# uci-cbcl/RP-Net

Hardware: AMD Instinct MI355X
Metric: support/query pairs/sec (fwd+bwd, 1-shot 256x256, T=5) (higher is better)
Workload: dtype f32

## Files before the change

### rpnet_amd/csrc/conv_wgrad_ring.hip

```cpp
#include <type_traits>

#include "common.h"
#include "lds_dma.h"
#include "split_bf16.h"

namespace rpnet {

using s16x4r = __attribute__((ext_vector_type(4))) short;
typedef __attribute__((address_space(3))) s16x4r lds_s16x4r_t;

template <int N, int I = 0, typename F>
__device__ __forceinline__ void static_for_r(F&& f) {
    if constexpr (I < N) {
        f(std::integral_constant<int, I>{});
        static_for_r<N, I + 1>(f);
    }
}

template <bool K64, int ABL = 0, int LA = 5, int NSY = 6, bool BI = false>
__global__ __launch_bounds__(256, 1) void conv_wgrad9_ring_kernel(const rpnet_conv_desc d, const unsigned short* __restrict__ dy,
                                                                   float* __restrict__ partial, const int M, const int Cin,
                                                                   const int Cout, const int tiles, const int tiles_n,
                                                                   const int ksplit, const int steps_per_split, const int lw,
                                                                   const int lh) {
    constexpr int NP = 2, BK = 32, RB = 128;
    constexpr int A_PLANE = BK * RB, A_STRIP = NP * A_PLANE;
    constexpr int NSX = 8, ZOFF = NSX * A_STRIP;
    constexpr int ZROW = 40, B_PLANE = 48 * RB, B_STAGE = NP * B_PLANE;
    constexpr int NS = NSY, BOFF = ZOFF + A_STRIP;
    static_assert(LA >= 2 && LA <= 5 && LA % NSY >= 2, "the DMAs of step st + LA must not land in a slot / stage that step st or st + 1 reads");
    __shared__ __attribute__((aligned(1024))) unsigned char smem[BOFF + NS * B_STAGE];
    RPNET_ASSERT_NO_CORESIDENCE(sizeof(smem));
    constexpr int PXS = K64 ? 64 : BK;

    const int t = threadIdx.x;
    const int lane = t & 63;
    const int wv = __builtin_amdgcn_readfirstlane(t >> 6);
    const int wm = wv >> 1, wn = wv & 1;
    int tile, z;
    const int xg = ksplit < 8 ? 8 / max(ksplit, 1) : 0;
    if ((ksplit & 7) == 0) {
        const int xcd = blockIdx.x & 7, j = blockIdx.x >> 3;
        const int jt = uni(j / tiles);
        z = jt * 8 + xcd;
        tile = j - jt * tiles;
    } else if (xg * ksplit == 8 && tiles % xg == 0) {
        const int xcd = blockIdx.x & 7, j = blockIdx.x >> 3;
        z = uni(xcd / xg);
        tile = (xcd - z * xg) * (tiles / xg) + j;
    } else {
        z = uni(blockIdx.x / tiles);
        tile = blockIdx.x - z * tiles;
    }
    const int tm = uni(tile / tiles_n), tn = tile - tm * tiles_n;
    const int cm0 = tm * 64, n0 = tn * 64;

    const int H = d.H, W = d.W;
    const unsigned short* src; int Cs, cc;
    if (cm0 < d.C0) { src = reinterpret_cast<const unsigned short*>(d.x0); Cs = d.C0; cc = cm0; }
    else { src = reinterpret_cast<const unsigned short*>(d.x1); Cs = d.C1; cc = cm0 - d.C0; }
    const size_t planex = (size_t)d.N * H * W * Cs, planey = (size_t)M * Cout;
    const int pbx = (int)(planex * 2), pby = (int)(planey * 2);

    const int total_steps = M / PXS;
    const int s_begin = z * steps_per_split;
    const int s_end = min(s_begin + steps_per_split, total_steps);
    const int lxb = lw - (K64 ? 6 : 5), xbm = (1 << lxb) - 1;
    auto q0_of = [&](const int s) {
        const int col = s >> lh, y = s & (H - 1);
        return ((((col >> lxb) << lh) + y) << lw) + (col & xbm) * PXS;
    };

    const srd_t rsx = make_srd(src, (K64 ? 1 : NP) * pbx), rsy = make_srd(dy, (K64 ? 1 : NP) * pby);
    const int x_slot1 = K64 ? BK * (Cs * 2) : pbx, y_slot1 = K64 ? BK * (Cout * 2) : pby;
    const __amdgpu_buffer_rsrc_t bix = __builtin_amdgcn_make_buffer_rsrc(const_cast<unsigned short*>(src), (short)0, (K64 ? 1 : NP) * pbx, 0x00020000);
    const __amdgpu_buffer_rsrc_t biy = __builtin_amdgcn_make_buffer_rsrc(const_cast<unsigned short*>(dy), (short)0, (K64 ? 1 : NP) * pby, 0x00020000);
    auto dma16 = [&](const bool is_x, const unsigned base, auto offc, const int voff, const int soff) {
        constexpr int OFF = decltype(offc)::value;
        if constexpr (BI) {
            auto* lp = (__attribute__((address_space(3))) void*)(smem + (base - lds_addr(smem)) + OFF);
            if (is_x) __builtin_amdgcn_raw_ptr_buffer_load_lds(bix, lp, 16, voff, soff, 0, 0);
            else __builtin_amdgcn_raw_ptr_buffer_load_lds(biy, lp, 16, voff, soff, 0, 0);
        } else if constexpr (OFF == 0) {
            lds_dma16(is_x ? rsx : rsy, base, voff, soff);
        } else {
            lds_dma16_at<OFF>(is_x ? rsx : rsy, base, voff, soff);
        }
    };
    const unsigned lds0 = lds_addr(smem);
    const unsigned ldsw = lds0 + 8 * wv * RB;
    const unsigned lds4 = lds0 + 32 * RB + (wv & 1) * B_PLANE;

    const int drow = lane >> 3;
    const int dcol = ((((lane >> 2) & 1) ^ ((lane >> 4) & 1)) << 6) | ((lane & 3) << 4);
    const int Cs2 = Cs * 2;
    const int xlane = drow * Cs2 + dcol;
    auto dma_x = [&](const int slot, const int rs) {
        if constexpr (ABL == 2 || ABL == 4) return;
        const int soff = (q0_of(rs) + 8 * wv) * Cs2 + cc * 2;
        const unsigned dst = ldsw + (slot & (NSX - 1)) * A_STRIP;
        dma16(true, dst, std::integral_constant<int, 0>{}, xlane, soff);
        dma16(true, dst, std::integral_constant<int, A_PLANE>{}, xlane, soff + x_slot1);
    };
    const int ylane = drow * (Cout * 2) + dcol, ylane_m1 = ylane - Cout * 2;
    auto dma_y = [&](auto stagec, const int st) {
        constexpr int stage = decltype(stagec)::value;
        constexpr int DST = BOFF + stage * B_STAGE;
        if constexpr (ABL == 2 || ABL == 4) return;
        const int rowb = q0_of(st) - 1 + 8 * wv;
        const bool neg = rowb < 0;
        const int soff = (neg ? 0 : rowb) * (Cout * 2) + n0 * 2;
        int voff = neg ? ylane_m1 : ylane;
        voff = rowb + drow < M ? voff : (int)0x80000000;
        const int soff1 = K64 ? (rowb + BK) * (Cout * 2) + n0 * 2 : soff + y_slot1;
        const int voff1 = K64 ? (rowb + BK + drow < M ? ylane : (int)0x80000000) : voff;
        dma16(false, ldsw, std::integral_constant<int, DST>{}, voff, soff);
        dma16(false, ldsw, std::integral_constant<int, DST + B_PLANE>{}, voff1, soff1);
    };
    auto dma_y5 = [&](auto stagec, const int st) {
        constexpr int stage = decltype(stagec)::value;
        constexpr int DST = BOFF + stage * B_STAGE;
        if constexpr (ABL == 2 || ABL == 4) return;
        const int rowb = q0_of(st) + 31 + (K64 ? wv * BK : 0);
        const int soff = rowb * (Cout * 2) + n0 * 2 + (K64 ? 0 : wv * y_slot1);
        const int voff = rowb + drow < M ? ylane : (int)0x80000000;
        dma16(false, lds4, std::integral_constant<int, DST>{}, voff, soff);
    };
    const int xlast = total_steps - 1;
    auto stc = [&](const int st) { return st < s_end ? st : s_end - 1; };
    auto xsc = [&](const int r) { return r < xlast ? r : xlast; };
    auto wait_all_but_one_step = [&]() {
        if constexpr (ABL == 2 || ABL == 4 || ABL >= 5) return;
        asm volatile("s_waitcnt vmcnt(%0)" ::"n"((LA - 2) * 4) : "memory");
    };

    {
        const u32x4 zero = {0u, 0u, 0u, 0u};
        *reinterpret_cast<u32x4*>(smem + ZOFF + t * 16) = zero;
        *reinterpret_cast<u32x4*>(smem + ZOFF + 4096 + t * 16) = zero;
        if (t < NS * NP * 8) {
            const int pl = t >> 3;
            *reinterpret_cast<u32x4*>(smem + BOFF + (pl / NP) * B_STAGE + (pl % NP) * B_PLANE + ZROW * RB + (t & 7) * 16) = zero;
        }
    }

    f32x16 acc[9];
#pragma unroll
    for (int a = 0; a < 9; ++a)
#pragma unroll
        for (int r = 0; r < 16; ++r) acc[a][r] = 0.f;

    const int g = lane >> 4, L = lane & 15;
    const int krow = 8 * (g >> 1) + (L >> 2);
    const int cbyte = (16 * (g & 1) + 4 * (L & 3)) * 2;
    const int a_off = krow * RB + (((wm ^ ((krow >> 1) & 1)) << 6) | cbyte);
    const unsigned char* const aptr = smem + a_off;
    int b_off[3];
#pragma unroll
    for (int kx = 0; kx < 3; ++kx) {
        const int r = krow + 2 - kx;
        b_off[kx] = BOFF + r * RB + (((wn ^ ((r >> 1) & 1)) << 6) | cbyte);
    }
    const int b_zero = BOFF + ZROW * RB + ((wn << 6) | cbyte);
    auto tr = [&](const unsigned char* p) -> s16x4r {
        return __builtin_amdgcn_ds_read_tr16_b64_v4i16((lds_s16x4r_t*)p);
    };

    struct ABase { const unsigned char* p[3]; };
    auto a_bases = [&](const int st) {
        const int y = st & (H - 1);
        const int o0 = y > 0 ? ((st - 1) & (NSX - 1)) * A_STRIP : ZOFF;
        const int o2 = y < H - 1 ? ((st + 1) & (NSX - 1)) * A_STRIP : ZOFF;
        ABase b;
        b.p[0] = aptr + o0;
        b.p[1] = aptr + (st & (NSX - 1)) * A_STRIP;
        b.p[2] = aptr + o2;
        return b;
    };

    s16x4r afr[2][3][NP][2], bfr[2][3][NP][2];
    if constexpr (ABL == 3 || ABL == 4) {
#pragma unroll
        for (int i = 0; i < 2 * 3 * NP * 2; ++i) {
            (&afr[0][0][0][0])[i] = s16x4r{(short)(lane + i), (short)(15360 + i), (short)lane, (short)i};
            (&bfr[0][0][0][0])[i] = s16x4r{(short)(lane * 3 + i), (short)(15361 + i), (short)(lane + 7), (short)(i * 5)};
        }
    }
    const unsigned char* bsel[2][3][2];
    const unsigned char* bconst[2][3][2];
#pragma unroll
    for (int s2 = 0; s2 < 2; ++s2)
#pragma unroll
        for (int kx = 0; kx < 3; ++kx)
#pragma unroll
            for (int e = 0; e < 2; ++e) bsel[s2][kx][e] = bconst[s2][kx][e] = smem + b_off[kx] + (16 * s2 + 4 * e) * RB;
    const unsigned char* const bzero = smem + b_zero;
    const bool lane_first = krow == 0, lane_last = krow == 11;
    auto b_addr = [&](auto sc, const int st) {
        constexpr int s = decltype(sc)::value;
        const int xb = (st >> lh) & xbm;
        if constexpr (s == 0) bsel[0][2][0] = (xb == 0 && lane_first) ? bzero : bconst[0][2][0];
        else bsel[1][0][1] = (xb == xbm && lane_last) ? bzero : bconst[1][0][1];
    };
    constexpr int NR = NP * 12, NMMA = (K64 ? 2 : nprod<NP>()) * 9;
    auto read_frag = [&](auto sc, auto kc, auto stagec, const ABase& ab) {
        constexpr int s = decltype(sc)::value, k = decltype(kc)::value, stage = decltype(stagec)::value;
        constexpr int grp = k / 12, r = (k - grp * 12) >> 1, e = k & 1;
        constexpr int pa = K64 ? grp : NP - 1 - grp, pb = grp;
        if constexpr (ABL == 3 || ABL == 4) return;
        if constexpr (r == 0 || r >= 4) {
            constexpr int ky = r == 0 ? 0 : r - 3;
            afr[s][ky][pa][e] = tr(ab.p[ky] + (pa * A_PLANE + (16 * s + 4 * e) * RB));
        } else {
            constexpr int kx = r - 1;
            constexpr bool sel = !K64 || (pb == 0 ? (s == 0 && kx == 2 && e == 0) : (s == 1 && kx == 0 && e == 1));
            bfr[s][kx][pb][e] = tr((sel ? bsel[s][kx][e] : bconst[s][kx][e]) + (stage * B_STAGE + pb * B_PLANE));
        }
    };
    auto frag = [](const s16x4r lo, const s16x4r hi) {
        return __builtin_bit_cast(bf16x8, __builtin_shufflevector(lo, hi, 0, 1, 2, 3, 4, 5, 6, 7));
    };
    auto mma_one = [&](auto sc, auto mc) {
        constexpr int s = decltype(sc)::value, m = decltype(mc)::value;
        constexpr int q = m / 9, tap = m - q * 9, ky = tap / 3, kx = tap - ky * 3;
        constexpr int pa = K64 ? q : prod_a<NP>(q), pb = K64 ? q : prod_b<NP>(q);
        acc[tap] = mma16<NP>(frag(afr[s][ky][pa][0], afr[s][ky][pa][1]), frag(bfr[s][kx][pb][0], bfr[s][kx][pb][1]), acc[tap]);
    };
    using I0 = std::integral_constant<int, 0>;
    using I1 = std::integral_constant<int, 1>;

    if (s_begin < s_end) {
        dma_x(s_begin - 1, s_begin > 0 ? s_begin - 1 : 0);
        dma_x(s_begin, s_begin);
        static_for_r<LA>([&](auto gc) {
            constexpr int gi = decltype(gc)::value;
            dma_x(s_begin + gi + 1, xsc(s_begin + gi + 1));
            dma_y(std::integral_constant<int, gi % NSY>{}, stc(s_begin + gi));
            if (wv < 2) dma_y5(std::integral_constant<int, gi % NSY>{}, stc(s_begin + gi));
        });
        wait_all_but_one_step();
        __builtin_amdgcn_s_barrier();
        ABase ab = a_bases(s_begin);
        b_addr(I0{}, s_begin);
        b_addr(I1{}, s_begin);
        static_for_r<NR>([&](auto kc) { read_frag(I0{}, kc, I0{}, ab); });

        const int g0 = s_begin + LA;
        int qa = q0_of(g0), qb = q0_of(g0 + 1);
        int yb = (g0 + 1) & (H - 1), xbb = ((g0 + 1) >> lh) & xbm;
        int xslot = ((g0 + 1) & (NSX - 1)) * A_STRIP;
        int cslot = (s_begin & (NSX - 1)) * A_STRIP;
        const int cx = 8 * wv * Cs2 + cc * 2;
        const int Cout2 = Cout * 2, c8 = 8 * wv - 1, cy = n0 * 2;
        const int c5 = 31 + (K64 ? wv * BK : 0), cy5 = cy + (K64 ? 0 : wv * y_slot1);
        const int col_next = PXS - W - (H - 1) * W, col_wrap = PXS - W;
        int sx = 0, sy = 0, sy5 = 0, rowb = 0, vy = ylane, y1 = 0, o0 = 0, o1 = 0, o2 = 0;
        unsigned dstx = 0;
        constexpr bool DMA_ON = !(ABL == 2 || ABL == 4);
        auto xa = [&]() { sx = qb * Cs2 + cx; dstx = ldsw + xslot; };
        auto xd0 = [&]() { if constexpr (DMA_ON) dma16(true, dstx, std::integral_constant<int, 0>{}, xlane, sx); };
        auto xd1 = [&]() { if constexpr (DMA_ON) dma16(true, dstx, std::integral_constant<int, A_PLANE>{}, xlane, sx + x_slot1); };
        auto ya1 = [&]() {
            rowb = qa + c8;
            vy = rowb < 0 ? ylane_m1 : ylane;
        };
        auto ya2 = [&]() { sy = max(rowb, 0) * Cout2 + cy; };
        auto yd0 = [&](auto stagec) {
            if constexpr (DMA_ON) dma16(false, ldsw, std::integral_constant<int, BOFF + decltype(stagec)::value * B_STAGE>{}, vy, sy);
        };
        auto yd1 = [&](auto stagec) {
            constexpr int DST = BOFF + decltype(stagec)::value * B_STAGE + B_PLANE;
            if constexpr (!DMA_ON) return;
            if constexpr (K64) dma16(false, ldsw, std::integral_constant<int, DST>{}, ylane, (rowb + BK) * Cout2 + cy);
            else dma16(false, ldsw, std::integral_constant<int, DST>{}, vy, sy + y_slot1);
        };
        auto y5a = [&]() { sy5 = (qa + c5) * Cout2 + cy5; };
        auto y5d = [&](auto stagec) {
            if constexpr (DMA_ON)
                if (wv < 2) dma16(false, lds4, std::integral_constant<int, BOFF + decltype(stagec)::value * B_STAGE>{}, ylane, sy5);
        };
        auto qs = [&]() { qa = qb; xslot = (xslot + A_STRIP) & (NSX * A_STRIP - 1); };
        auto adv = [&]() {
            qb += W;
            yb += 1;
            if (yb == H) {
                const bool last = xbb == xbm;
                yb = 0;
                qb += last ? col_wrap : col_next;
                xbb = last ? 0 : xbb + 1;
            }
        };
        auto ab1 = [&](const int st) { y1 = (st + 1) & (H - 1); o1 = (cslot + A_STRIP) & (NSX * A_STRIP - 1); };
        auto ab2 = [&]() { o0 = y1 > 0 ? cslot : ZOFF; o2 = y1 < H - 1 ? ((o1 + A_STRIP) & (NSX * A_STRIP - 1)) : ZOFF; };
        auto ab3 = [&]() { ab.p[0] = aptr + o0; ab.p[1] = aptr + o1; ab.p[2] = aptr + o2; cslot = o1; };
        constexpr int M0 = K64 ? 6 : 1;
        auto step = [&](auto kc4, const int st) {
            constexpr int K = decltype(kc4)::value;
            using SK = std::integral_constant<int, K>;
            using SN = std::integral_constant<int, (K + 1) % NSY>;
            using SD = std::integral_constant<int, (K + LA) % NSY>;
            static_for_r<NMMA>([&](auto mc) {
                constexpr int m = decltype(mc)::value;
                mma_one(I0{}, mc);
                __builtin_amdgcn_sched_barrier(0);
                if constexpr (m < NR) {
                    read_frag(I1{}, mc, SK{}, ab);
                    __builtin_amdgcn_sched_barrier(0);
                }
                if constexpr (NR > NMMA && m < NR - NMMA) {
                    read_frag(I1{}, std::integral_constant<int, NMMA + m>{}, SK{}, ab);
                    __builtin_amdgcn_sched_barrier(0);
                }
                if constexpr (m == M0) xa();
                if constexpr (m == M0 + 2) xd0();
                if constexpr (m == M0 + 4) xd1();
                if constexpr (m == NMMA - 3) ab1(st);
                if constexpr (m == NMMA - 2) ab2();
                if constexpr (m == NMMA - 1) { ab3(); b_addr(I0{}, st + 1); }
                if constexpr (m == M0 || m == M0 + 2 || m == M0 + 4 || m >= NMMA - 3) __builtin_amdgcn_sched_barrier(0);
            });
            static_for_r<NMMA>([&](auto mc) {
                constexpr int m = decltype(mc)::value;
                mma_one(I1{}, mc);
                __builtin_amdgcn_sched_barrier(0);
                if constexpr (m < NR) {
                    read_frag(I0{}, mc, SN{}, ab);
                    __builtin_amdgcn_sched_barrier(0);
                }
                if constexpr (NR > NMMA && m < NR - NMMA) {
                    read_frag(I0{}, std::integral_constant<int, NMMA + m>{}, SN{}, ab);
                    __builtin_amdgcn_sched_barrier(0);
                }
                if constexpr (m == M0) ya1();
                if constexpr (m == M0 + 1) ya2();
                if constexpr (m == M0 + 2) yd0(SD{});
                if constexpr (m == M0 + 4) yd1(SD{});
                if constexpr (m == M0 + 5) y5a();
                if constexpr (m == M0 + 6) y5d(SD{});
                if constexpr (m == M0 + 8) qs();
                if constexpr (m == M0 + 9) adv();
                if constexpr (m == NMMA - 1) b_addr(I1{}, st + 1);
                if constexpr ((m >= M0 && m <= M0 + 9) || m == NMMA - 1) __builtin_amdgcn_sched_barrier(0);
            });
            wait_all_but_one_step();
            if constexpr (ABL != 6) __builtin_amdgcn_s_barrier();
        };
        for (int st = s_begin; st < s_end; st += NSY) {
            bool done = false;
            static_for_r<NSY>([&](auto kc) {
                constexpr int k = decltype(kc)::value;
                if (!done) {
                    step(kc, st + k);
                    done = st + k + 1 >= s_end;
                }
            });
            if (done) break;
        }
        asm volatile("s_waitcnt vmcnt(0)" ::: "memory");
        __builtin_amdgcn_s_barrier();
    }
    if (z >= ksplit) return;
    const int li = lane & 31, h = lane >> 5;
    constexpr int SW = 36;
    float* slab = reinterpret_cast<float*>(smem) + wv * 32 * SW;
#pragma unroll
    for (int tap = 0; tap < 9; ++tap) {
#pragma unroll
        for (int r = 0; r < 16; ++r) slab[((r & 3) + 8 * (r >> 2) + 4 * h) * SW + li] = acc[tap][r];
        __builtin_amdgcn_wave_barrier();
        float* out = partial + ((size_t)(z * 9 + tap) * Cin + cm0 + wm * 32) * Cout + n0 + wn * 32;
#pragma unroll
        for (int q = 0; q < 4; ++q) {
            const int gidx = q * 64 + lane, rr = gidx >> 3, c4 = gidx & 7;
            *reinterpret_cast<f32x4*>(out + (size_t)rr * Cout + c4 * 4) = *reinterpret_cast<const f32x4*>(&slab[rr * SW + c4 * 4]);
        }
        __builtin_amdgcn_wave_barrier();
    }
}

static int ilog2r(int v) {
    int l = 0;
    while ((1 << l) < v) ++l;
    return (1 << l) == v ? l : -1;
}

bool conv_wgrad9_ring_ok(const rpnet_conv_desc* d, int M, int sps9) {
    const int lw = ilog2r(d->W), lh = ilog2r(d->H);
    if (lw < 0 || lh < 0 || d->upsample) return false;
    if (d->split_planes == 2) return d->W >= 32;
    return d->split_planes == 1 && d->W >= 64 && M % 64 == 0 && sps9 % 2 == 0;
}

int conv_wgrad9_ring(const rpnet_conv_desc* d, const void* dy, float* part9, int M, int Cin, int Cout, int ks9, int sps9,
                     hipStream_t s) {
    const int tiles_n9 = Cout / 64, tiles9 = (Cin / 64) * tiles_n9;
    const int lw = ilog2r(d->W), lh = ilog2r(d->H);
    const unsigned short* dys = (const unsigned short*)dy;
    const int abl = (d->tune >> 8) & 7;
#define RPNET_W9R(K6, A, SPS)                                                                                                   \
    hipLaunchKernelGGL((conv_wgrad9_ring_kernel<K6, A>), dim3(tiles9 * ks9), dim3(256), 0, s, *d, dys, part9, M, Cin, Cout, tiles9, \
                       tiles_n9, ks9, SPS, lw, lh)
    if (d->split_planes == 2 && (d->tune & 255) == 18) {
        hipLaunchKernelGGL((conv_wgrad9_ring_kernel<false, 0, 5, 6, true>), dim3(tiles9 * ks9), dim3(256), 0, s, *d, dys, part9, M, Cin, Cout, tiles9,
                           tiles_n9, ks9, sps9, lw, lh);
    } else if (d->split_planes == 2 && (d->tune & 255) == 17) {
        hipLaunchKernelGGL((conv_wgrad9_ring_kernel<false, 0, 3, 4>), dim3(tiles9 * ks9), dim3(256), 0, s, *d, dys, part9, M, Cin, Cout, tiles9,
                           tiles_n9, ks9, sps9, lw, lh);
    } else if (d->split_planes == 2) {
        if (abl == 2) RPNET_W9R(false, 2, sps9);
        else if (abl == 3) RPNET_W9R(false, 3, sps9);
        else if (abl == 4) RPNET_W9R(false, 4, sps9);
        else if (abl == 5) RPNET_W9R(false, 5, sps9);
        else if (abl == 6) RPNET_W9R(false, 6, sps9);
        else RPNET_W9R(false, 0, sps9);
    } else {
        RPNET_W9R(true, 0, sps9 / 2);
    }
#undef RPNET_W9R
    return check_launch("conv_wgrad9_ring");
}

}
```

Measured before the change: 503.6.

## Extend ring weight-gradient conv kernel to 16-wide images via two-rows-per-step mode

Adds a NARROW template mode to the ring wgrad kernel so layers with W=16 (previously rejected, falling back to another path) can use it. Each 32-pixel step covers two image rows, and the vertical-neighbor fragments are read from the other half of the adjacent strip. Horizontal edge zeroing is fixed per lane, and the row indexing runs over H/2 steps. This brings the ring kernel's LDS reuse and DMA pipelining to the small deep layers, at the cost of more complex address logic that could be wrong at boundaries.

```diff
diff --git a/rpnet_amd/csrc/conv_wgrad_ring.hip b/rpnet_amd/csrc/conv_wgrad_ring.hip
--- a/rpnet_amd/csrc/conv_wgrad_ring.hip
+++ b/rpnet_amd/csrc/conv_wgrad_ring.hip
@@ -17,7 +17,7 @@
     }
 }
 
-template <bool K64, int ABL = 0, int LA = 5, int NSY = 6, bool BI = false>
+template <bool K64, int ABL = 0, int LA = 5, int NSY = 6, bool BI = false, bool NARROW = false>
 __global__ __launch_bounds__(256, 1) void conv_wgrad9_ring_kernel(const rpnet_conv_desc d, const unsigned short* __restrict__ dy,
                                                                    float* __restrict__ partial, const int M, const int Cin,
                                                                    const int Cout, const int tiles, const int tiles_n,
@@ -28,6 +28,7 @@
     constexpr int NSX = 8, ZOFF = NSX * A_STRIP;
     constexpr int ZROW = 40, B_PLANE = 48 * RB, B_STAGE = NP * B_PLANE;
     constexpr int NS = NSY, BOFF = ZOFF + A_STRIP;
+    static_assert(!(NARROW && K64), "the two-rows-per-step form exists on two planes only");
     static_assert(LA >= 2 && LA <= 5 && LA % NSY >= 2, "the DMAs of step st + LA must not land in a slot / stage that step st or st + 1 reads");
     __shared__ __attribute__((aligned(1024))) unsigned char smem[BOFF + NS * B_STAGE];
     RPNET_ASSERT_NO_CORESIDENCE(sizeof(smem));
@@ -56,6 +57,7 @@
     const int cm0 = tm * 64, n0 = tn * 64;
 
     const int H = d.H, W = d.W;
+    const int HS = NARROW ? H >> 1 : H;
     const unsigned short* src; int Cs, cc;
     if (cm0 < d.C0) { src = reinterpret_cast<const unsigned short*>(d.x0); Cs = d.C0; cc = cm0; }
     else { src = reinterpret_cast<const unsigned short*>(d.x1); Cs = d.C1; cc = cm0 - d.C0; }
@@ -65,8 +67,9 @@
     const int total_steps = M / PXS;
     const int s_begin = z * steps_per_split;
     const int s_end = min(s_begin + steps_per_split, total_steps);
-    const int lxb = lw - (K64 ? 6 : 5), xbm = (1 << lxb) - 1;
+    const int lxb = NARROW ? 0 : lw - (K64 ? 6 : 5), xbm = (1 << lxb) - 1;
     auto q0_of = [&](const int s) {
+        if constexpr (NARROW) return s * PXS;
         const int col = s >> lh, y = s & (H - 1);
         return ((((col >> lxb) << lh) + y) << lw) + (col & xbm) * PXS;
     };
@@ -168,9 +171,9 @@
 
     struct ABase { const unsigned char* p[3]; };
     auto a_bases = [&](const int st) {
-        const int y = st & (H - 1);
+        const int y = st & (HS - 1);
         const int o0 = y > 0 ? ((st - 1) & (NSX - 1)) * A_STRIP : ZOFF;
-        const int o2 = y < H - 1 ? ((st + 1) & (NSX - 1)) * A_STRIP : ZOFF;
+        const int o2 = y < HS - 1 ? ((st + 1) & (NSX - 1)) * A_STRIP : ZOFF;
         ABase b;
         b.p[0] = aptr + o0;
         b.p[1] = aptr + (st & (NSX - 1)) * A_STRIP;
@@ -196,8 +199,16 @@
             for (int e = 0; e < 2; ++e) bsel[s2][kx][e] = bconst[s2][kx][e] = smem + b_off[kx] + (16 * s2 + 4 * e) * RB;
     const unsigned char* const bzero = smem + b_zero;
     const bool lane_first = krow == 0, lane_last = krow == 11;
+    if constexpr (NARROW) {
+#pragma unroll
+        for (int s2 = 0; s2 < 2; ++s2) {
+            bsel[s2][2][0] = lane_first ? bzero : bconst[s2][2][0];
+            bsel[s2][0][1] = lane_last ? bzero : bconst[s2][0][1];
+        }
+    }
     auto b_addr = [&](auto sc, const int st) {
         constexpr int s = decltype(sc)::value;
+        if constexpr (NARROW) return;
         const int xb = (st >> lh) & xbm;
         if constexpr (s == 0) bsel[0][2][0] = (xb == 0 && lane_first) ? bzero : bconst[0][2][0];
         else bsel[1][0][1] = (xb == xbm && lane_last) ? bzero : bconst[1][0][1];
@@ -210,7 +221,11 @@
         if constexpr (ABL == 3 || ABL == 4) return;
         if constexpr (r == 0 || r >= 4) {
             constexpr int ky = r == 0 ? 0 : r - 3;
-            afr[s][ky][pa][e] = tr(ab.p[ky] + (pa * A_PLANE + (16 * s + 4 * e) * RB));
+            if constexpr (NARROW && ky != 1) {
+                constexpr int sp = ky == 0 ? s : s + 1;
+                afr[s][ky][pa][e] = tr(ab.p[sp] + (pa * A_PLANE + (16 * (1 - s) + 4 * e) * RB));
+            } else
+                afr[s][ky][pa][e] = tr(ab.p[ky] + (pa * A_PLANE + (16 * s + 4 * e) * RB));
         } else {
             constexpr int kx = r - 1;
             constexpr bool sel = !K64 || (pb == 0 ? (s == 0 && kx == 2 && e == 0) : (s == 1 && kx == 0 && e == 1));
@@ -247,7 +262,7 @@
 
         const int g0 = s_begin + LA;
         int qa = q0_of(g0), qb = q0_of(g0 + 1);
-        int yb = (g0 + 1) & (H - 1), xbb = ((g0 + 1) >> lh) & xbm;
+        int yb = (g0 + 1) & (HS - 1), xbb = ((g0 + 1) >> lh) & xbm;
         int xslot = ((g0 + 1) & (NSX - 1)) * A_STRIP;
         int cslot = (s_begin & (NSX - 1)) * A_STRIP;
         const int cx = 8 * wv * Cs2 + cc * 2;
@@ -281,6 +296,10 @@
         };
         auto qs = [&]() { qa = qb; xslot = (xslot + A_STRIP) & (NSX * A_STRIP - 1); };
         auto adv = [&]() {
+            if constexpr (NARROW) {
+                qb += PXS;
+                return;
+            }
             qb += W;
             yb += 1;
             if (yb == H) {
@@ -290,8 +309,8 @@
                 xbb = last ? 0 : xbb + 1;
             }
         };
-        auto ab1 = [&](const int st) { y1 = (st + 1) & (H - 1); o1 = (cslot + A_STRIP) & (NSX * A_STRIP - 1); };
-        auto ab2 = [&]() { o0 = y1 > 0 ? cslot : ZOFF; o2 = y1 < H - 1 ? ((o1 + A_STRIP) & (NSX * A_STRIP - 1)) : ZOFF; };
+        auto ab1 = [&](const int st) { y1 = (st + 1) & (HS - 1); o1 = (cslot + A_STRIP) & (NSX * A_STRIP - 1); };
+        auto ab2 = [&]() { o0 = y1 > 0 ? cslot : ZOFF; o2 = y1 < HS - 1 ? ((o1 + A_STRIP) & (NSX * A_STRIP - 1)) : ZOFF; };
         auto ab3 = [&]() { ab.p[0] = aptr + o0; ab.p[1] = aptr + o1; ab.p[2] = aptr + o2; cslot = o1; };
         constexpr int M0 = K64 ? 6 : 1;
         auto step = [&](auto kc4, const int st) {
@@ -384,10 +403,15 @@
     return (1 << l) == v ? l : -1;
 }
 
+static bool ring_narrow(const rpnet_conv_desc* d) {
+    const int tv = d->tune & 255;
+    return d->split_planes == 2 && d->W == 16 && d->H >= 2 && tv != 17 && tv != 18 && ((d->tune >> 8) & 7) == 0;
+}
+
 bool conv_wgrad9_ring_ok(const rpnet_conv_desc* d, int M, int sps9) {
     const int lw = ilog2r(d->W), lh = ilog2r(d->H);
     if (lw < 0 || lh < 0 || d->upsample) return false;
-    if (d->split_planes == 2) return d->W >= 32;
+    if (d->split_planes == 2) return d->W >= 32 || ring_narrow(d);
     return d->split_planes == 1 && d->W >= 64 && M % 64 == 0 && sps9 % 2 == 0;
 }
 
@@ -400,7 +424,10 @@
 #define RPNET_W9R(K6, A, SPS)                                                                                                   \
     hipLaunchKernelGGL((conv_wgrad9_ring_kernel<K6, A>), dim3(tiles9 * ks9), dim3(256), 0, s, *d, dys, part9, M, Cin, Cout, tiles9, \
                        tiles_n9, ks9, SPS, lw, lh)
-    if (d->split_planes == 2 && (d->tune & 255) == 18) {
+    if (ring_narrow(d)) {
+        hipLaunchKernelGGL((conv_wgrad9_ring_kernel<false, 0, 5, 6, false, true>), dim3(tiles9 * ks9), dim3(256), 0, s, *d, dys, part9, M, Cin, Cout,
+                           tiles9, tiles_n9, ks9, sps9, lw, lh - 1);
+    } else if (d->split_planes == 2 && (d->tune & 255) == 18) {
         hipLaunchKernelGGL((conv_wgrad9_ring_kernel<false, 0, 5, 6, true>), dim3(tiles9 * ks9), dim3(256), 0, s, *d, dys, part9, M, Cin, Cout, tiles9,
                            tiles_n9, ks9, sps9, lw, lh);
     } else if (d->split_planes == 2 && (d->tune & 255) == 17) {
```

After: 505.5, median of 5. Within noise of the previous version (+0.4%).
